# amirhajibabaei/AutoForce

Hardware: AMD Instinct MI355X
Metric: MD-step atoms*steps/sec (SGPR predict: NL + descriptors + K_nm + E/F/stress + covloss); `value`: a Langevin MD loop on the device, every step from the forces of the one before (sgpr_md_run; --steps dependent steps between two fences); `value_resident_frames`: steps over independent frames resident i (higher is better)
Workload: dtype f64

## Files before the change

autoforce_amd/csrc/descriptor.hip:

```cpp
#include "sgpr_internal.h"
#include "gemm_tile.inc"

__constant__ HarmCoef c_hc;

void upload_harm_coef(const HarmCoef &hc) { (void)hipMemcpyToSymbol(HIP_SYMBOL(c_hc), &hc, sizeof(HarmCoef)); }

#define SQRT2 1.4142135623730951
typedef double v4d __attribute__((ext_vector_type(4)));

__device__ __forceinline__ void wave_sync()
{
    __builtin_amdgcn_fence(__ATOMIC_RELEASE, "wavefront");
    __builtin_amdgcn_wave_barrier();
    __builtin_amdgcn_fence(__ATOMIC_ACQUIRE, "wavefront");
}

__device__ __forceinline__ double uniform(double v)
{
    const int lo = __builtin_amdgcn_readfirstlane(__double2loint(v));
    const int hi = __builtin_amdgcn_readfirstlane(__double2hiint(v));
    return __hiloint2double(hi, lo);
}

template <typename T>
// ... 231 lines not shown
template <int LMAX, int NMAX, int ST>
__device__ __forceinline__ int species_in_use(const DescArgs &a)
{
    if constexpr (LMAX == 3 && NMAX == 3 && ST <= 4) return ST;
    else return a.S;
}

template <bool ENV>
__device__ __forceinline__ void load_neighbor(const DescArgs &a, int gi, int ia, int t, const double *pi,
                                              const double *cell, double r[3], int &s, int &j)
{
    if constexpr (ENV) {
        const int64_t e = a.env_ptr[ia] + t;
        r[0] = a.env_r[3 * e]; r[1] = a.env_r[3 * e + 1]; r[2] = a.env_r[3 * e + 2];
        s = a.env_slot[e];
        j = -1;
    } else {
        const size_t e = (size_t)gi * a.maxnn + t;
        j = a.nbr_j[e];
        const int code = a.nbr_shift[e];
        const double s0 = (double)(int)(int8_t)(code & 0xff);
        const double s1 = (double)(int)(int8_t)((code >> 8) & 0xff);
        const double s2 = (double)(int)(int8_t)((code >> 16) & 0xff);
#pragma unroll
        for (int k = 0; k < 3; k++)
            r[k] = a.pos[3 * (size_t)j + k] - pi[k] + (s0 * cell[k] + s1 * cell[3 + k] + s2 * cell[6 + k]);
        s = (code >> 24) & 0xff;
    }
}

template <int NMAX>
__device__ __forceinline__ void radial_ex(double d, double u, double rc, double irc, double ex, double *f, double &g,
                                          double &dg)
{
    const double ud = u * d;
    const double step = ud < rc ? 1.0 : 0.0;
    const double qq = 1.0 - ud * irc;
    const double cut = step * qq * qq;
    const double dcut = step * (-2.0 * qq * irc) * u;
    g = cut * ex;
    dg = dcut * ex - d * g;
    const double rho = d * d;
    double pw = g;
#pragma unroll
    for (int n = 0; n <= NMAX; n++) { f[n] = pw; pw *= rho; }
}

template <int NMAX>
__device__ __forceinline__ void radial(double d, double u, double rc, double *f, double &g, double &dg, double &ex)
{
    ex = exp(-0.5 * d * d);
    radial_ex<NMAX>(d, u, rc, 1.0 / rc, ex, f, g, dg);
}

template <int LMAX, int NMAX>
struct WaveLds {
    static constexpr int L1 = LMAX + 1, N1 = NMAX + 1, LL = L1 * L1, LLP = LL + 1, NSLOT = N1 * LL;
    static constexpr int CH = 48;
    static constexpr int TILE_D = CH * N1 + CH * LLP;
    static constexpr int CHS = 64;
    static constexpr bool SWZ = LL == 16;
    static constexpr int RS = SWZ ? LL : (LL | 1);
    static __device__ __forceinline__ int rot(int row) { return (row ^ (row >> 4)) & 15; }
    static __device__ __forceinline__ int at(int row, int k) { return SWZ ? row * RS + (k ^ rot(row)) : row * RS + k; }
};

template <int LMAX, int NMAX, int ST, bool ENV>
__global__ __launch_bounds__(256) void desc_fwd_kernel(DescArgs a)
{
    using WL = WaveLds<LMAX, NMAX>;
    constexpr int N1 = WL::N1, LL = WL::LL, LLP = WL::LLP, NSLOT = WL::NSLOT;
    constexpr int SPL = (NSLOT + 63) / 64;
    extern __shared__ double smem[];
    const int wave = threadIdx.x >> 6, lane = threadIdx.x & 63;
    const int ia = blockIdx.x * 4 + wave;
    if (ia >= a.N) return;
    const int gi = a.first + ia * a.stride;
    constexpr int CH = WL::CH;
    const int perwave = WL::TILE_D + ST * NSLOT + 64 / 2;
    double *fl = smem + (size_t)wave * perwave;
    double *Yl = fl + CH * N1;
    double *cl = Yl + CH * LLP;
    int *sl = (int *)(cl + ST * NSLOT);

    int nn;
    double pi[3] = {0, 0, 0}, cell[9];
    if constexpr (ENV) {
        nn = (int)(a.env_ptr[ia + 1] - a.env_ptr[ia]);
    } else {
        nn = a.nn[gi];
#pragma unroll
        for (int k = 0; k < 3; k++) pi[k] = a.pos[3 * (size_t)gi + k];
#pragma unroll
        for (int k = 0; k < 9; k++) cell[k] = a.cell[k];
    }

    bool shear = false;
    if (nn > CH) {
        bool near = false;
        for (int t0 = 0; t0 < nn; t0 += 64) {
            const int t = t0 + lane;
            if (t < nn) {
                double r[3]; int s, j;
                load_neighbor<ENV>(a, gi, ia, t, pi, cell, r, s, j);
                const double u = unit_of<ST>(a, s);
                const double tol = SGPR_TINY_ANGLE * fabs(r[2] / u);
                near |= (fabs(r[0] / u) < tol) && (fabs(r[1] / u) < tol);
            }
        }
        shear = __any(near);
    }

    double acc[ST][SPL];
#pragma unroll
    for (int s = 0; s < ST; s++)
#pragma unroll
        for (int k = 0; k < SPL; k++) acc[s][k] = 0.0;

    for (int t0 = 0; t0 < nn; t0 += CH) {
        const int cnt = min(CH, nn - t0);
        const int t = lane < cnt ? t0 + lane : nn;
        wave_sync();
        double r[3] = {1.0, 0.0, 0.0};
        int s = 0, j = 0;
        if (t < nn) load_neighbor<ENV>(a, gi, ia, t, pi, cell, r, s, j);
        const double u = unit_of<ST>(a, s);
        const double iu = 1.0 / u;
        const double x = r[0] * iu, y = r[1] * iu, z = r[2] * iu;
        if (nn <= CH) {
            const double tol = SGPR_TINY_ANGLE * fabs(z);
            shear = __any(t < nn && fabs(x) < tol && fabs(y) < tol);
        }
        const double ang = shear ? SGPR_TINY_ANGLE : 0.0;
        if (t < nn) {
            const double d = sqrt(x * x + y * y + z * z);
            double f[N1], g, dg, ex;
            radial<NMAX>(d, u, a.rc, f, g, dg, ex);
            if constexpr (!ENV) {
                if (a.prec) {
                    double2 *dst = (double2 *)(a.prec + ((size_t)gi * a.maxnn + t) * 4);
                    dst[0] = make_double2(r[0], r[1]);
                    dst[1] = make_double2(r[2], ex);
                }
            }
            double Y[LL];
            Harm<LMAX> h;
            h.eval(x, y - ang * z, ang * y + z, Y);
#pragma unroll
            for (int n = 0; n < N1; n++) fl[lane * N1 + n] = f[n];
#pragma unroll
            for (int k = 0; k < LL; k++) Yl[lane * LLP + k] = Y[k];
            sl[lane] = s;
        }
        wave_sync();
        const int sv = t < nn ? s : ST;
        const int sprev = __shfl_up(sv, 1, 64);
        const bool sorted = !ENV && !__any(lane > 0 && lane < cnt && sprev > sv);
        if (sorted) {
            int beg = 0;
#pragma unroll
            for (int q = 0; q < ST; q++) {
                const int end = beg + __popcll(__ballot(t < nn && s == q));
#pragma unroll 4
                for (int tt = beg; tt < end; tt++) {
#pragma unroll
                    for (int k = 0; k < SPL; k++) {
                        const int slot = lane + 64 * k;
                        if (SPL * 64 == NSLOT || slot < NSLOT)
                            acc[q][k] += fl[tt * N1 + slot / LL] * Yl[tt * LLP + slot % LL];
                    }
                }
                beg = end;
            }
        } else {
#pragma unroll 4
            for (int tt = 0; tt < cnt; tt++) {
                const int s = __builtin_amdgcn_readfirstlane(sl[tt]);
#pragma unroll
                for (int k = 0; k < SPL; k++) {
                    const int slot = lane + 64 * k;
                    if (SPL * 64 == NSLOT || slot < NSLOT) {
                        const double v = fl[tt * N1 + slot / LL] * Yl[tt * LLP + slot % LL];
#pragma unroll
                        for (int q = 0; q < ST; q++)
                            if (s == q) acc[q][k] += v;
                    }
                }
            }
        }
    }
    wave_sync();
#pragma unroll
    for (int s = 0; s < ST; s++)
#pragma unroll
        for (int k = 0; k < SPL; k++) {
            const int slot = lane + 64 * k;
            if (SPL * 64 == NSLOT || slot < NSLOT) {
                cl[s * NSLOT + slot] = acc[s][k];
                if (a.C && s < a.S) a.C[(size_t)ia * a.CS + s * NSLOT + slot] = acc[s][k];
            }
        }
    wave_sync();
    double nrm2 = 0.0;
    constexpr int L1 = LMAX + 1;
    constexpr int UMAX = ST * N1;
    constexpr int MAXP = ((UMAX * (UMAX + 1)) / 2 + 63) / 64;
    const int npair = a.Dc / L1;
    double pv[MAXP][L1];
#pragma unroll
    for (int k = 0; k < MAXP; k++) {
        const int pr = lane + 64 * k;
#pragma unroll
        for (int l = 0; l < L1; l++) pv[k][l] = 0.0;
        if (pr < npair) {
            const PackEntry p0 = a.pack[pr * L1];
            const double *cu = cl + (p0.u / N1) * NSLOT + (p0.u % N1) * LL;
            const double *cv = cl + (p0.v / N1) * NSLOT + (p0.v % N1) * LL;
#pragma unroll
            for (int l = 0; l < L1; l++) {
                double sacc = 0.0;
#pragma unroll
                for (int mm = 0; mm < 2 * l + 1; mm++) sacc += cu[l * l + mm] * cv[l * l + mm];
                pv[k][l] = sacc * a.pack[pr * L1 + l].coef;
                nrm2 += pv[k][l] * pv[k][l];
            }
        }
    }
    nrm2 = wave_sum(nrm2);
    const double nrm = sqrt(nrm2);
    const double inv = nn > 0 ? 1.0 / (nrm + SGPR_EPS) : 0.0;
#pragma unroll
    for (int k = 0; k < MAXP; k++) {
        const int pr = lane + 64 * k;
        if (pr < npair) {
#pragma unroll
            for (int l = 0; l < L1; l++) a.Pn[(size_t)ia * a.Dpad + pr * L1 + l] = pv[k][l] * inv;
        }
    }
    for (int e = a.Dc + lane; e < a.Dpad; e += 64) a.Pn[(size_t)ia * a.Dpad + e] = 0.0;
    if (lane == 0) {
        a.norm[ia] = nn > 0 ? nrm : 0.0;
        if (a.shear) a.shear[ia] = shear ? 1 : 0;
    }
}

#define NL_SORT_MAX 256
#ifndef NL_STEPS
#define NL_STEPS 4
#endif

struct NlArgs {
    const NlGrid *grid;
    const int *bin_of, *kslot, *bin_count;
    int cap;
    const BinRec *b_rec;
    const BinAux *b_aux;
    int *nn, *nn_local, *nn_raw, *nbr_j, *nbr_shift, *aux;
    unsigned short *T;
    int t_stride;
    int *stat;
    const int *flag;
    double rc_list;
    int *ncand, *cand_j, *cand_code, *cidx;
    unsigned long long *hm;
    int hmw;
};

#ifdef SGPR_PHASE_STAMPS
#define PHASE_STAMP(K) if (a.stamps && lane == 0) a.stamps[(size_t)ia * 8 + (K)] = (long long)__builtin_amdgcn_s_memtime()
#else
#define PHASE_STAMP(K)
#endif

template <int LMAX, int NMAX, int ST>
struct FwdLds {
    using WL = WaveLds<LMAX, NMAX>;
    static constexpr int CH = WL::CHS;
    static constexpr int BINL = NL_SORT_MAX + NL_SORT_MAX / 2, HIT0 = BINL + 2 * 64;
    static constexpr int NLV = HIT0 + 4 * CH;
    static constexpr int FWV = CH * WL::N1 + CH * WL::RS;
    static constexpr int P4V = ST * WL::NSLOT + 16;
    static constexpr int RA = (NLV > FWV ? (NLV > P4V ? NLV : P4V) : (FWV > P4V ? FWV : P4V));
    static constexpr int PW = RA;
};

template <int LMAX, int NMAX, int ST>
__global__ __launch_bounds__(256, 4) void nl_fwd_kernel(DescArgs a, NlArgs n)
{
    using WL = WaveLds<LMAX, NMAX>;
    using FL = FwdLds<LMAX, NMAX, ST>;
    constexpr int N1 = WL::N1, LL = WL::LL, NSLOT = WL::NSLOT, CH = WL::CHS;
    constexpr int UC = ST * N1, CBS = (UC + 15) / 16, RBL = (LL + 15) / 16;
    extern __shared__ double smem[];
    const int wave = __builtin_amdgcn_readfirstlane(threadIdx.x >> 6), lane = threadIdx.x & 63;
    const int ia = xcd_quad((int)blockIdx.x, (int)gridDim.x, a.xq) * 4 + wave;
    if (ia >= a.N) return;
    const int i = a.first + ia * a.stride;
    double *wbase = smem + (size_t)wave * FL::PW;
    double *RA = wbase;
    unsigned long long *keys = (unsigned long long *)RA;
    int *hq = (int *)(RA + NL_SORT_MAX);
    int4 *binl = (int4 *)(RA + FL::BINL);
    double *hit0 = RA + FL::HIT0;
    double *fl = RA;
    double *Yl = fl + CH * N1;
    double *cl = RA;

    PHASE_STAMP(0);
    const int cap = n.cap, maxnn = a.maxnn;
    double h[9];
#pragma unroll
    for (int k = 0; k < 9; k++) h[k] = a.cell[k];
    const double xi = uniform(a.pos[3 * (size_t)i]), yi = uniform(a.pos[3 * (size_t)i + 1]), zi = uniform(a.pos[3 * (size_t)i + 2]);
    const int ki = __builtin_amdgcn_readfirstlane(n.kslot[i]);
    const bool ghost = ki < 0;
    const unsigned long long lt = lane == 0 ? 0ull : (~0ull >> (64 - lane));
    const bool rebuild = __builtin_amdgcn_readfirstlane(*n.flag) != 0;
    int ncand = 0;
    int j_first = 0, cd_first = 0;
    if (rebuild) {
        const NlGrid g = *n.grid;
        const int bi = __builtin_amdgcn_readfirstlane(n.bin_of[i]);
        int wi0 = 0, wi1 = 0, wi2 = 0;
        if (ki >= 0 && ki < cap) {
            const BinAux own = n.b_aux[(size_t)bi * cap + ki];
            wi0 = own.w0; wi1 = own.w1; wi2 = own.w2;
        }
        auto fdiv = [](int q, float inv) { return (int)(((float)q + 0.5f) * inv); };
        const float i_n2 = 1.0f / (float)g.nb[2], i_n1 = 1.0f / (float)g.nb[1];
        const int bq = fdiv(bi, i_n2);
        const int b2 = bi - bq * g.nb[2];
        const int b0 = fdiv(bq, i_n1);
        const int b1 = bq - b0 * g.nb[1];
        const int w0 = 2 * g.rng[0] + 1, w1 = 2 * g.rng[1] + 1, w2 = 2 * g.rng[2] + 1;
        const float i_w2 = 1.0f / (float)w2, i_w1 = 1.0f / (float)w1;
        const double r_n0 = 1.0 / g.nb[0], r_n1 = 1.0 / g.nb[1], r_n2 = 1.0 / g.nb[2];
        const int nbox = w0 * w1 * w2;
        const bool t_ok = n.T != nullptr && (long long)nbox * cap <= (long long)n.t_stride && cap <= 4096 && maxnn <= 65535 &&
                          ki < cap && !ghost;
        if (n.T != nullptr && !t_ok && ki < cap && !ghost && lane == 0)
            atomicMax(&n.stat[2], cap <= 4096 && maxnn <= 65535 ? nbox * cap : 0x7fffffff);
        const int grp = lane >> 4, s16 = lane & 15;
        const double rl2 = n.rc_list * n.rc_list;
        int base = 0;
        auto consume = [&](bool valid, const BinRec &rec, const BinAux &ax, int code, int q, int k) {
            bool hit = false;
            int f0 = 0, f1 = 0, f2 = 0;
            if (valid) {
                f0 = (int)(int8_t)(code & 0xff) - ax.w0 + wi0;
                f1 = (int)(int8_t)((code >> 8) & 0xff) - ax.w1 + wi1;
                f2 = (int)(int8_t)((code >> 16) & 0xff) - ax.w2 + wi2;
                const double dx = rec.x - xi + (f0 * h[0] + f1 * h[3] + f2 * h[6]);
                const double dy = rec.y - yi + (f0 * h[1] + f1 * h[4] + f2 * h[7]);
                const double dz = rec.z - zi + (f0 * h[2] + f1 * h[5] + f2 * h[8]);
                hit = dx * dx + dy * dy + dz * dz < rl2 && !(rec.idx == i && f0 == 0 && f1 == 0 && f2 == 0);
            }
            const unsigned long long m = __ballot(hit);
            if (hit) {
                const int slot = base + __popcll(m & lt);
                const int j = rec.idx, sj = ax.slot;
                const unsigned img = (unsigned)((f0 + 128) & 0xff) << 16 | (unsigned)((f1 + 128) & 0xff) << 8 |
                                     (unsigned)((f2 + 128) & 0xff);
                const unsigned long long key = ((unsigned long long)(unsigned)j << 40) | ((unsigned long long)img << 16) |
                                               ((unsigned long long)(unsigned)sj << 12) | (unsigned)(slot & 0xfff);
                if (max(max(abs(f0), abs(f1)), abs(f2)) > 127) atomicMax(&n.stat[3], 1);
                if (slot < NL_SORT_MAX) {
                    keys[slot] = key;
                    hq[slot] = (q << 12) | k;
                } else if (slot < maxnn) {
                    const size_t e = (size_t)i * maxnn + slot;
                    n.cand_j[e] = j;
                    n.cand_code[e] = (f0 & 0xff) | ((f1 & 0xff) << 8) | ((f2 & 0xff) << 16) | (sj << 24);
                    n.aux[e] = 0;
                    if (t_ok) {
                        n.aux[e] = q * cap + k;
                        n.T[(size_t)j * n.t_stride + (size_t)(nbox - 1 - q) * cap + ki] = (unsigned short)slot;
                    }
                }
            }
            base += __popcll(m);
        };
        constexpr int STEPS = NL_STEPS;
        double tb[3];
#pragma unroll
        for (int k = 0; k < 3; k++) {
            const double fk = xi * g.inv[k] + yi * g.inv[3 + k] + zi * g.inv[6 + k];
            const double uk = (fk - floor(fk)) * g.nb[k] - (k == 0 ? b0 : k == 1 ? b1 : b2);
            tb[k] = g.rng[k] > 0 ? fmin(fmax(uk, 0.0), 1.0) : 0.0;
        }
        const double rl2_skip = rl2 * (1.0 + 1e-9);
        for (int q0 = 0; q0 < (ghost ? 0 : nbox); q0 += 64) {
            int nbin_l = 0, code_l = 0, cnt_l = 0;
            bool keep = false;
            {
                const int q = q0 + lane;
                if (q < nbox) {
                    const int qa = fdiv(q, i_w2), qb = fdiv(qa, i_w1);
                    const int o2 = q - qa * w2 - g.rng[2], o1 = qa - qb * w1 - g.rng[1], o0 = qb - g.rng[0];
                    const int t0 = b0 + o0, t1 = b1 + o1, t2 = b2 + o2;
                    const int c0 = (int)floor((double)t0 * r_n0 + 1e-9), c1 = (int)floor((double)t1 * r_n1 + 1e-9),
                              c2 = (int)floor((double)t2 * r_n2 + 1e-9);
                    nbin_l = ((t0 - c0 * g.nb[0]) * g.nb[1] + (t1 - c1 * g.nb[1])) * g.nb[2] + (t2 - c2 * g.nb[2]);
                    code_l = (c0 & 0xff) | ((c1 & 0xff) << 8) | ((c2 & 0xff) << 16);
                    cnt_l = min(n.bin_count[(size_t)nbin_l * SGPR_BIN_STRIDE], cap);
                    const double g0 = (o0 > 0 ? o0 - tb[0] : o0 < 0 ? tb[0] - o0 - 1.0 : 0.0) * g.w[0];
                    const double g1 = (o1 > 0 ? o1 - tb[1] : o1 < 0 ? tb[1] - o1 - 1.0 : 0.0) * g.w[1];
                    const double g2 = (o2 > 0 ? o2 - tb[2] : o2 < 0 ? tb[2] - o2 - 1.0 : 0.0) * g.w[2];
                    const double gm = fmax(g0, fmax(g1, g2));
                    const double lb2 = g.ortho ? g0 * g0 + g1 * g1 + g2 * g2 : gm * gm;
                    keep = cnt_l > 0 && lb2 < rl2_skip;
                }
            }
            const unsigned long long km = __ballot(keep);
            const int nlist = __popcll(km);
            wave_sync();
            if (keep) binl[__popcll(km & lt)] = make_int4(nbin_l, code_l, cnt_l, q0 + lane);
            wave_sync();
            const int nsteps = (nlist + 3) >> 2;
            for (int u0 = 0; u0 < nsteps; u0 += STEPS) {
                int nbin[STEPS], code[STEPS], cnt[STEPS], qq[STEPS], cmax = 0;
#pragma unroll
                for (int u = 0; u < STEPS; u++) {
                    const int e = 4 * (u0 + u) + grp;
                    const int4 bb = binl[e < nlist ? e : 0];
                    nbin[u] = bb.x; code[u] = bb.y; qq[u] = bb.w;
                    cnt[u] = e < nlist ? bb.z : 0;
                    cmax = max(cmax, cnt[u]);
                }
                for (int s0 = 0; __any(s0 < cmax); s0 += 16) {
                    BinRec rec[STEPS];
                    BinAux ax[STEPS];
#pragma unroll
                    for (int u = 0; u < STEPS; u++) {
                        const size_t e = (size_t)nbin[u] * cap + (s0 + s16 < cnt[u] ? s0 + s16 : 0);
                        rec[u] = n.b_rec[e];
                        ax[u] = n.b_aux[e];
                    }
#pragma unroll
                    for (int u = 0; u < STEPS; u++)
                        if (__any(s0 + s16 < cnt[u])) consume(s0 + s16 < cnt[u], rec[u], ax[u], code[u], qq[u], s0 + s16);
                }
            }
        }
        PHASE_STAMP(1);
        const int ns = min(base, NL_SORT_MAX);
        wave_sync();
        if (ns <= 64) {
            unsigned long long key = lane < ns ? keys[lane] : ~0ull;
#pragma unroll
            for (int k2s = 2; k2s <= 64; k2s <<= 1)
#pragma unroll
                for (int j2 = k2s >> 1; j2 > 0; j2 >>= 1) {
                    const unsigned lo = __shfl_xor((unsigned)key, j2, 64), hi = __shfl_xor((unsigned)(key >> 32), j2, 64);
                    const unsigned long long other = ((unsigned long long)hi << 32) | lo;
                    const bool lower = (lane & j2) == 0, up = (lane & k2s) == 0;
                    const bool take_min = lower == up;
                    key = take_min ? (other < key ? other : key) : (other > key ? other : key);
                }
            wave_sync();
            if (lane < ns) keys[lane] = key;
        } else {
            int np2 = 1;
            while (np2 < ns) np2 <<= 1;
            for (int t = ns + lane; t < np2; t += 64) keys[t] = ~0ull;
            wave_sync();
            for (int k2s = 2; k2s <= np2; k2s <<= 1)
                for (int j2 = k2s >> 1; j2 > 0; j2 >>= 1) {
                    for (int t = lane; t < np2; t += 64) {
                        const int p = t ^ j2;
                        if (p > t) {
                            const unsigned long long a0 = keys[t], a1 = keys[p];
                            const bool up = (t & k2s) == 0;
                            if ((a0 > a1) == up) { keys[t] = a1; keys[p] = a0; }
                        }
                    }
                    wave_sync();
                }
        }
        wave_sync();
        ncand = base < maxnn ? base : maxnn;
        for (int c = lane; c < ns && c < maxnn; c += 64) {
            const unsigned long long key = keys[c];
            const unsigned img = (unsigned)(key >> 16) & 0xffffffu;
            const int f0 = (int)((img >> 16) & 0xff) - 128, f1 = (int)((img >> 8) & 0xff) - 128, f2 = (int)(img & 0xff) - 128,
                      sj = (int)(key >> 12) & 0xf, j = (int)(key >> 40);
            const size_t e = (size_t)i * maxnn + c;
            n.cand_j[e] = j;
            n.cand_code[e] = (f0 & 0xff) | ((f1 & 0xff) << 8) | ((f2 & 0xff) << 16) | (sj << 24);
            int hs = 0;
            if (t_ok) {
                const int hv = hq[(int)key & 0xfff];
                const int qv = hv >> 12, kk = hv & 0xfff;
                hs = qv * cap + kk;
                n.T[(size_t)j * n.t_stride + (size_t)(nbox - 1 - qv) * cap + ki] = (unsigned short)c;
            }
            n.aux[e] = hs;
        }
        if (lane == 0) {
            n.ncand[i] = ncand;
            n.nn_raw[ia] = base;
        }
        if (ncand > NL_SORT_MAX) __threadfence();
        PHASE_STAMP(2);
    } else {
        const int nc_v = n.ncand[i];
        if (lane < maxnn) {
            const size_t e = (size_t)i * maxnn + lane;
            j_first = n.cand_j[e];
            cd_first = n.cand_code[e];
        }
        ncand = __builtin_amdgcn_readfirstlane(nc_v);
        if (lane == 0) n.nn_raw[ia] = ncand;
    }
    const double rc2_lo = a.rc * a.rc * (1.0 - 1e-14), rc2_hi = a.rc * a.rc * (1.0 + 1e-14);
    int nn = 0;
    bool near = false;
    for (int c0 = 0; c0 < ncand; c0 += 64) {
        const int c = c0 + lane;
        bool hit = false;
        int j = 0, cd = 0;
        double r0 = 1.0, r1 = 0.0, r2 = 0.0;
        if (c < ncand) {
            if (rebuild && c < NL_SORT_MAX) {
                const unsigned long long key = keys[c];
                const unsigned img = (unsigned)(key >> 16) & 0xffffffu;
                const int f0 = (int)((img >> 16) & 0xff) - 128, f1 = (int)((img >> 8) & 0xff) - 128, f2 = (int)(img & 0xff) - 128;
                j = (int)(key >> 40);
                cd = (f0 & 0xff) | ((f1 & 0xff) << 8) | ((f2 & 0xff) << 16) | (((int)(key >> 12) & 0xf) << 24);
            } else if (!rebuild && c0 == 0) {
                j = j_first; cd = cd_first;
            } else {
                const size_t e = (size_t)i * maxnn + c;
                j = n.cand_j[e];
                cd = n.cand_code[e];
            }
            const int f0 = (int)(int8_t)(cd & 0xff), f1 = (int)(int8_t)((cd >> 8) & 0xff), f2 = (int)(int8_t)((cd >> 16) & 0xff);
            r0 = a.pos[3 * (size_t)j] - xi + (f0 * h[0] + f1 * h[3] + f2 * h[6]);
            r1 = a.pos[3 * (size_t)j + 1] - yi + (f0 * h[1] + f1 * h[4] + f2 * h[7]);
            r2 = a.pos[3 * (size_t)j + 2] - zi + (f0 * h[2] + f1 * h[5] + f2 * h[8]);
            const double d2 = r0 * r0 + r1 * r1 + r2 * r2;
            hit = d2 < rc2_lo || (d2 < rc2_hi && sqrt(d2) < a.rc);
        }
        const unsigned long long m = __ballot(hit);
        if (lane == 0) n.hm[(size_t)i * n.hmw + (c0 >> 6)] = m;
        if (hit) {
            const int t = nn + __popcll(m & lt);
            const int sj = (cd >> 24) & 0xff;
            const size_t e = (size_t)i * maxnn + t;
            n.nbr_j[e] = j;
            n.nbr_shift[e] = cd;
            n.cidx[e] = c;
            double *dst = t < CH ? hit0 + 4 * t : nullptr;
            if (dst) { dst[0] = r0; dst[1] = r1; dst[2] = r2; dst[3] = __hiloint2double(0, sj); }
            const double tol = SGPR_TINY_ANGLE * fabs(r2);
            near |= (fabs(r0) < tol) && (fabs(r1) < tol);
        }
        nn += __popcll(m);
    }
    for (int w = (ncand + 63) / 64 + lane; w < n.hmw; w += 64) n.hm[(size_t)i * n.hmw + w] = 0ull;
    const bool shear = __any(near);
    if (lane == 0) {
        n.nn[i] = nn;
        n.nn_local[ia] = nn;
    }
    wave_sync();
    double h0r[3] = {1.0, 0.0, 0.0};
    int h0s = 0;
    if (lane < min(nn, CH)) {
        h0r[0] = hit0[4 * lane]; h0r[1] = hit0[4 * lane + 1]; h0r[2] = hit0[4 * lane + 2];
        h0s = __double2loint(hit0[4 * lane + 3]);
    }
    if (nn > CH) __threadfence();
    PHASE_STAMP(3);
    v4d D[RBL][CBS];
#pragma unroll
    for (int rb = 0; rb < RBL; rb++)
#pragma unroll
        for (int cb = 0; cb < CBS; cb++) D[rb][cb] = (v4d){0.0, 0.0, 0.0, 0.0};
    const double ang = shear ? SGPR_TINY_ANGLE : 0.0;
    for (int t0 = 0; t0 < nn; t0 += CH) {
        const int cnt = min(CH, nn - t0);
        const bool on = lane < cnt;
        const int t = t0 + lane;
        double r[3] = {1.0, 0.0, 0.0};
        int s = 0;
        if (on) {
            if (t0 == 0) { r[0] = h0r[0]; r[1] = h0r[1]; r[2] = h0r[2]; s = h0s; }
            else {
                const size_t e = (size_t)i * maxnn + t;
                const int j = n.nbr_j[e];
                const int cd = n.nbr_shift[e];
                const int f0 = (int)(int8_t)(cd & 0xff), f1 = (int)(int8_t)((cd >> 8) & 0xff), f2 = (int)(int8_t)((cd >> 16) & 0xff);
                s = (cd >> 24) & 0xff;
                r[0] = a.pos[3 * (size_t)j] - xi + (f0 * h[0] + f1 * h[3] + f2 * h[6]);
                r[1] = a.pos[3 * (size_t)j + 1] - yi + (f0 * h[1] + f1 * h[4] + f2 * h[7]);
                r[2] = a.pos[3 * (size_t)j + 2] - zi + (f0 * h[2] + f1 * h[5] + f2 * h[8]);
            }
        }
        const double u = unit_of<ST>(a, s);
        const double iu = inv_unit_of<ST>(a, s);
        const double x = r[0] * iu, y = r[1] * iu, z = r[2] * iu;
        const double d = sqrt(x * x + y * y + z * z);
        double f[N1], gg, dg;
        const double ex = exp(-0.5 * d * d);
        radial_ex<NMAX>(d, u, a.rc, a.irc, ex, f, gg, dg);
        double Y[LL];
        Harm<LMAX> hm;
        hm.eval(x, y - ang * z, ang * y + z, Y);
        if (on && a.prec) {
            double2 *dst = (double2 *)(a.prec + ((size_t)i * maxnn + t) * 4);
            dst[0] = make_double2(r[0], r[1]);
            dst[1] = make_double2(r[2], ex);
        }
        wave_sync();
#pragma unroll
        for (int q = 0; q < N1; q++) fl[lane * N1 + q] = on ? f[q] : 0.0;
#pragma unroll
        for (int k = 0; k < LL; k++) Yl[WL::at(lane, k)] = on ? Y[k] : 0.0;
        const int sv = on ? s : -1;
        wave_sync();
        for (int g16 = 0; g16 < cnt; g16 += 16) {
            double av[4][RBL], bv[4][CBS];
#pragma unroll
            for (int q = 0; q < 4; q++) {
                const int tr = g16 + 4 * q + (lane >> 4);
                const int st = __shfl(sv, tr, 64);
#pragma unroll
                for (int rb = 0; rb < RBL; rb++) {
                    const int lm = 16 * rb + (lane & 15);
                    av[q][rb] = (RBL * 16 == LL || lm < LL) ? Yl[WL::at(tr, lm < LL ? lm : 0)] : 0.0;
                }
#pragma unroll
                for (int cb = 0; cb < CBS; cb++) {
                    const int c = 16 * cb + (lane & 15);
                    const double fv = fl[tr * N1 + (c < UC ? c % N1 : 0)];
                    bv[q][cb] = (c < UC && st == c / N1) ? fv : 0.0;
                }
            }
#pragma unroll
            for (int q = 0; q < 4; q++)
#pragma unroll
                for (int rb = 0; rb < RBL; rb++)
#pragma unroll
                    for (int cb = 0; cb < CBS; cb++)
                        D[rb][cb] = __builtin_amdgcn_mfma_f64_16x16x4f64(av[q][rb], bv[q][cb], D[rb][cb], 0, 0, 0);
        }
    }
    wave_sync();
    PHASE_STAMP(4);
    constexpr int L1 = LMAX + 1;
    constexpr int UMAX = ST * N1;
    constexpr bool PMF = UMAX <= 16;
    constexpr int CLS = PMF ? LL + 1 : LL;
#pragma unroll
    for (int rb = 0; rb < RBL; rb++)
#pragma unroll
        for (int cb = 0; cb < CBS; cb++)
#pragma unroll
            for (int q = 0; q < 4; q++) {
                const int lm = 16 * rb + (lane >> 4) + 4 * q, c = 16 * cb + (lane & 15);
                if ((RBL * 16 == LL || lm < LL) && (CBS * 16 == UC || c < UC)) {
                    const int idx = (c / N1) * NSLOT + (c % N1) * LL + lm;
                    cl[PMF ? c * CLS + lm : idx] = D[rb][cb][q];
                }
            }
    wave_sync();
    if (a.C)
        for (int idx = lane; idx < species_in_use<LMAX, NMAX, ST>(a) * NSLOT; idx += 64)
            a.C[(size_t)ia * a.CS + idx] = cl[PMF ? (idx / LL) * CLS + idx % LL : idx];
    double nrm2 = 0.0;
    const int npair = a.Dc / L1;
    if constexpr (PMF) {
        const int Ur = species_in_use<LMAX, NMAX, ST>(a) * N1, vch = lane & 15;
        double cf[L1][4];
        int eidx[4];
#pragma unroll
        for (int r = 0; r < 4; r++) {
            const int u = (lane >> 4) + 4 * r;
            const bool keep = u <= vch && vch < Ur;
            eidx[r] = keep ? (u * Ur - (u * (u - 1)) / 2 + (vch - u)) * L1 : -1;
#pragma unroll
            for (int l = 0; l < L1; l++) cf[l][r] = keep ? a.pack[eidx[r] + l].coef : 0.0;
        }
        v4d P[L1];
#pragma unroll
        for (int l = 0; l < L1; l++) {
            P[l] = (v4d){0.0, 0.0, 0.0, 0.0};
#pragma unroll
            for (int ks = 0; ks < (2 * l + 4) / 4; ks++) {
                const int kk = 4 * ks + (lane >> 4);
                const double av = (vch < Ur && kk < 2 * l + 1) ? cl[vch * CLS + l * l + kk] : 0.0;
                P[l] = __builtin_amdgcn_mfma_f64_16x16x4f64(av, av, P[l], 0, 0, 0);
            }
        }
#pragma unroll
        for (int l = 0; l < L1; l++)
#pragma unroll
            for (int r = 0; r < 4; r++) {
                const double pvv = P[l][r] * cf[l][r];
                cf[l][r] = pvv;
                nrm2 += pvv * pvv;
            }
        nrm2 = wave_sum(nrm2);
        const double nrm = sqrt(nrm2);
        const double inv = nn > 0 ? 1.0 / (nrm + SGPR_EPS) : 0.0;
#pragma unroll
        for (int r = 0; r < 4; r++)
            if (eidx[r] >= 0) {
#pragma unroll
                for (int l = 0; l < L1; l++) a.Pn[(size_t)ia * a.Dpad + eidx[r] + l] = cf[l][r] * inv;
            }
        for (int e = a.Dc + lane; e < a.Dpad; e += 64) a.Pn[(size_t)ia * a.Dpad + e] = 0.0;
        if (lane == 0) {
            a.norm[ia] = nn > 0 ? nrm : 0.0;
            if (a.shear) a.shear[ia] = shear ? 1 : 0;
        }
        PHASE_STAMP(5);
        return;
    }
    constexpr int MAXP = ((UMAX * (UMAX + 1)) / 2 + 63) / 64;
    double pv[MAXP][L1];
#pragma unroll
    for (int k = 0; k < MAXP; k++) {
        const int pr = lane + 64 * k;
#pragma unroll
        for (int l = 0; l < L1; l++) pv[k][l] = 0.0;
        if (pr < npair) {
            const PackEntry p0 = a.pack[pr * L1];
            const double *cu = cl + (p0.u / N1) * NSLOT + (p0.u % N1) * LL;
            const double *cv = cl + (p0.v / N1) * NSLOT + (p0.v % N1) * LL;
#pragma unroll
            for (int l = 0; l < L1; l++) {
                double sacc = 0.0;
#pragma unroll
                for (int mm = 0; mm < 2 * l + 1; mm++) sacc += cu[l * l + mm] * cv[l * l + mm];
                pv[k][l] = sacc * a.pack[pr * L1 + l].coef;
                nrm2 += pv[k][l] * pv[k][l];
            }
        }
    }
    nrm2 = wave_sum(nrm2);
    const double nrm = sqrt(nrm2);
    const double inv = nn > 0 ? 1.0 / (nrm + SGPR_EPS) : 0.0;
#pragma unroll
    for (int k = 0; k < MAXP; k++) {
        const int pr = lane + 64 * k;
        if (pr < npair) {
#pragma unroll
            for (int l = 0; l < L1; l++) a.Pn[(size_t)ia * a.Dpad + pr * L1 + l] = pv[k][l] * inv;
        }
    }
    for (int e = a.Dc + lane; e < a.Dpad; e += 64) a.Pn[(size_t)ia * a.Dpad + e] = 0.0;
    if (lane == 0) {
        a.norm[ia] = nn > 0 ? nrm : 0.0;
        if (a.shear) a.shear[ia] = shear ? 1 : 0;
    }
    PHASE_STAMP(5);
}

template <int LMAX, int NMAX>
struct RevDims {
    static constexpr int N1 = NMAX + 1, L1 = LMAX + 1, LL = L1 * L1, NSLOT = N1 * LL;
    static constexpr int KS = (N1 + 3) / 4;
    static constexpr int CB = (LL + 15) / 16;
    static constexpr int CH = WaveLds<LMAX, NMAX>::CHS, RB = CH / 16;
    static constexpr bool SKEW = LL == 16;
    static constexpr int SP = LL | 1;
    static constexpr int STAGE = SKEW ? CH * LL + CH / 2 : CH * SP;
    static __device__ __forceinline__ int at(int row) { return SKEW ? row * LL + (row >> 1) : row * SP; }
    static constexpr int FS = 8 * KS + 1;
};

template <int LMAX, int NMAX, int ST>
static int rev_region_doubles(int Dpad)
{
    using RD = RevDims<LMAX, NMAX>;
    const int UT = ST * RD::N1;
    const int dc = ST * RD::NSLOT + (ST <= 4 ? UT * UT * RD::L1 : Dpad);
    int r = RD::STAGE;
    if (RD::CH * RD::FS > r) r = RD::CH * RD::FS;
    if (12 * RD::CH > r) r = 12 * RD::CH;
    if (dc > r) r = dc;
    return (r + 1) & ~1;
}

template <int LMAX, int NMAX, int ST, bool GATHER, bool ROWS, bool COV = false>
__global__ __launch_bounds__(256, 4) void desc_rev_kernel(DescArgs a, GemmArgs gc, int n_cov)
{
    extern __shared__ double smem[];
    const int S_use = species_in_use<LMAX, NMAX, ST>(a);
    if constexpr (COV) {
        if ((int)blockIdx.x < n_cov) {
            using GL = GemmLds<EPI_ROWSQ, 1, 16>;
            gemm_tile_body<EPI_ROWSQ, 1, 16>(gc, (int)blockIdx.x, smem, smem + GL::NBUF * GL::ASZ);
            return;
        }
    }
    const int bx = COV ? (int)blockIdx.x - n_cov : (int)blockIdx.x;
    const int nbx = COV ? (int)gridDim.x - n_cov : (int)gridDim.x;
    const double *const rows_aw = ROWS ? a.rows_aw : nullptr;
    using RD = RevDims<LMAX, NMAX>;
    constexpr int N1 = RD::N1, L1 = RD::L1, LL = RD::LL, NSLOT = RD::NSLOT;
    constexpr int KS = RD::KS, CB = RD::CB, CH = RD::CH, RB = RD::RB, SP = RD::SP, FS = RD::FS;
    constexpr int SPL = (NSLOT + 63) / 64;
    constexpr int WPW = SGPR_REV_WPW(ST);
    __shared__ double vred[4][9];
    const int wave = __builtin_amdgcn_readfirstlane(threadIdx.x >> 6), lane = threadIdx.x & 63;
    const int qd = xcd_quad(bx, nbx, a.xq);
    const int ia = qd * WPW + wave;
    const bool active = ia < a.N;
    const int perwave = ST * NSLOT + a.rsz + CH / 8;
    double *dcl = smem + (size_t)wave * perwave;
    double *R = dcl + ST * NSLOT;
// ... 541 lines not shown
```

Baseline: 50.77 million.

## Compact bin-overflow neighbor scan via prefix sums and hoist candidate-list loads

During neighbor-list rebuild, each bin is now scanned once for its first 16 slots. Overflow entries beyond 16 are flattened across all bins with a wave prefix sum and a binary search, so every lane processes one leftover record. This avoids the old loop that ran to the largest bin count, where many lanes sat idle. Separately, the cached candidate list, ncand, kslot and the rebuild flag are loaded unconditionally at kernel entry so their latency overlaps the position loads. The cost is extra loads on rebuild steps and a binary search per overflow element.

```diff
diff --git a/autoforce_amd/csrc/descriptor.hip b/autoforce_amd/csrc/descriptor.hip
--- a/autoforce_amd/csrc/descriptor.hip
+++ b/autoforce_amd/csrc/descriptor.hip
@@ -557,22 +557,32 @@
     int *hq = (int *)(RA + NL_SORT_MAX);
     int4 *binl = (int4 *)(RA + FL::BINL);
     double *hit0 = RA + FL::HIT0;
+    int *lsum = (int *)hit0;
     double *fl = RA;
     double *Yl = fl + CH * N1;
     double *cl = RA;
 
     PHASE_STAMP(0);
     const int cap = n.cap, maxnn = a.maxnn;
+    int nc_v = 0, j_first = 0, cd_first = 0;
+    if (lane < maxnn) {
+        const size_t e = (size_t)i * maxnn + lane;
+        int zero = 0;
+        asm("" : "+v"(zero));
+        nc_v = n.ncand[i + zero];
+        j_first = n.cand_j[e];
+        cd_first = n.cand_code[e];
+    }
     double h[9];
 #pragma unroll
     for (int k = 0; k < 9; k++) h[k] = a.cell[k];
     const double xi = uniform(a.pos[3 * (size_t)i]), yi = uniform(a.pos[3 * (size_t)i + 1]), zi = uniform(a.pos[3 * (size_t)i + 2]);
-    const int ki = __builtin_amdgcn_readfirstlane(n.kslot[i]);
+    const int ki_v = n.kslot[i], flag_v = *n.flag;
+    const int ki = __builtin_amdgcn_readfirstlane(ki_v);
     const bool ghost = ki < 0;
     const unsigned long long lt = lane == 0 ? 0ull : (~0ull >> (64 - lane));
-    const bool rebuild = __builtin_amdgcn_readfirstlane(*n.flag) != 0;
+    const bool rebuild = __builtin_amdgcn_readfirstlane(flag_v) != 0;
     int ncand = 0;
-    int j_first = 0, cd_first = 0;
     if (rebuild) {
         const NlGrid g = *n.grid;
         const int bi = __builtin_amdgcn_readfirstlane(n.bin_of[i]);
@@ -668,33 +678,55 @@
             }
             const unsigned long long km = __ballot(keep);
             const int nlist = __popcll(km);
+            int lsum_l = keep ? max(cnt_l - 16, 0) : 0;
+#pragma unroll
+            for (int d = 1; d < 64; d <<= 1) {
+                const int up = __shfl_up(lsum_l, d, 64);
+                if (lane >= d) lsum_l += up;
+            }
+            const int nleft = __builtin_amdgcn_readlane(lsum_l, 63);
             wave_sync();
-            if (keep) binl[__popcll(km & lt)] = make_int4(nbin_l, code_l, cnt_l, q0 + lane);
+            if (keep) {
+                const int e = __popcll(km & lt);
+                binl[e] = make_int4(nbin_l, code_l, cnt_l, q0 + lane);
+                lsum[e] = lsum_l;
+            }
             wave_sync();
             const int nsteps = (nlist + 3) >> 2;
             for (int u0 = 0; u0 < nsteps; u0 += STEPS) {
-                int nbin[STEPS], code[STEPS], cnt[STEPS], qq[STEPS], cmax = 0;
+                int nbin[STEPS], code[STEPS], cnt[STEPS], qq[STEPS];
 #pragma unroll
                 for (int u = 0; u < STEPS; u++) {
                     const int e = 4 * (u0 + u) + grp;
                     const int4 bb = binl[e < nlist ? e : 0];
                     nbin[u] = bb.x; code[u] = bb.y; qq[u] = bb.w;
                     cnt[u] = e < nlist ? bb.z : 0;
-                    cmax = max(cmax, cnt[u]);
-                }
-                for (int s0 = 0; __any(s0 < cmax); s0 += 16) {
-                    BinRec rec[STEPS];
-                    BinAux ax[STEPS];
-#pragma unroll
-                    for (int u = 0; u < STEPS; u++) {
-                        const size_t e = (size_t)nbin[u] * cap + (s0 + s16 < cnt[u] ? s0 + s16 : 0);
-                        rec[u] = n.b_rec[e];
-                        ax[u] = n.b_aux[e];
-                    }
-#pragma unroll
-                    for (int u = 0; u < STEPS; u++)
-                        if (__any(s0 + s16 < cnt[u])) consume(s0 + s16 < cnt[u], rec[u], ax[u], code[u], qq[u], s0 + s16);
-                }
+                }
+                BinRec rec[STEPS];
+                BinAux ax[STEPS];
+#pragma unroll
+                for (int u = 0; u < STEPS; u++) {
+                    const size_t e = (size_t)nbin[u] * cap + (s16 < cnt[u] ? s16 : 0);
+                    rec[u] = n.b_rec[e];
+                    ax[u] = n.b_aux[e];
+                }
+#pragma unroll
+                for (int u = 0; u < STEPS; u++)
+                    if (__any(s16 < cnt[u])) consume(s16 < cnt[u], rec[u], ax[u], code[u], qq[u], s16);
+            }
+            for (int t0 = 0; t0 < nleft; t0 += 64) {
+                const int t = t0 + lane;
+                const bool valid = t < nleft;
+                int e = 0;
+#pragma unroll
+                for (int s = 32; s > 0; s >>= 1)
+                    if (valid && e + s <= nlist && lsum[e + s - 1] <= t) e += s;
+                const int4 bb = binl[valid ? e : 0];
+                const int k = valid ? 16 + t - (e > 0 ? lsum[e - 1] : 0) : 0;
+                const size_t er = (size_t)bb.x * cap + k;
+                const BinRec rec = n.b_rec[er];
+                const BinAux ax = n.b_aux[er];
+                consume(valid, rec, ax, bb.y, bb.w, k);
             }
         }
         PHASE_STAMP(1);
@@ -758,12 +790,6 @@
         if (ncand > NL_SORT_MAX) __threadfence();
         PHASE_STAMP(2);
     } else {
-        const int nc_v = n.ncand[i];
-        if (lane < maxnn) {
-            const size_t e = (size_t)i * maxnn + lane;
-            j_first = n.cand_j[e];
-            cd_first = n.cand_code[e];
-        }
         ncand = __builtin_amdgcn_readfirstlane(nc_v);
         if (lane == 0) n.nn_raw[ia] = ncand;
     }
```

Result: no change. 50.66 million (-0.2%).
